# lsl036/STM-Multifrontal-QR-Factorization-Empowered-by-GCN

Measured on AMD Instinct MI355X. Metric: numerical-factorization GFLOP/s, higher is better.
Workload: dtype f64; 1 GPU; xenon1_colamd_standin: m=49248 n=49248 nnz=1258432 fronts=686 flops/step=5.029e+11, ordering default (COLAMD: qrtest without an ordering argument) (stand-in for xenon1.mtx, absent from the reference checkout); inputs=values resident in HBM, factors left in HBM, parallelism=replica x1, levels=16, retries=0

## Files before the change

### stm-multifrontal-qr-factorization-empowered-by-gcn_amd/csrc/stmmqr_update.hip

```cpp
#include <hip/hip_ext.h>
#include "stmmqr_kdev.h"
#include "stmmqr_knobs.h"


__global__ __launch_bounds__(NT) void k_update(DevCtx c, const int *__restrict__ flist, const int *__restrict__ plist, int cb0)
{
    extern __shared__ double dyn_lds[];
    const int f = flist[blockIdx.y];
    const int p = plist[blockIdx.y];
    const FrontSym s = c.fs[f];
    if (p >= s.npanels) return;
    const PanelDesc *pd = &c.fnum[f].pd[STM_PDI(p)];
    const int cbg = cb0 + (int)blockIdx.x * (1 + c.cbskip);
    const int c0 = pd->pc0 + cbg * BN;
    if (c0 >= s.fn) return;
    double *Tw = c.Tws + (long long)STM_TSLOT(c.tslot[f], p) * STM_NB * STM_NB;
    if (pd->t_deferred) {
        const bool first = (cbg == 0) || (c.cbskip > 0 && blockIdx.x == 0);
        dev_update_block(c.Farena + s.foff, s.ld, pd->pg1, pd->pt - pd->pg1, pd->pk1, pd->pnb, pd->pdiag, nullptr, c0,
                         min(BN, s.fn - c0), dyn_lds, c.Tau + s.rp + pd->pk1, first ? Tw : nullptr,
                         (first && c.Tall) ? c.Tall + (long long)(s.tpan + p) * STM_NB * STM_NB : nullptr);
        return;
    }
    dev_update_block(c.Farena + s.foff, s.ld, pd->pg1, pd->pt - pd->pg1, pd->pk1, pd->pnb, pd->pdiag, Tw, c0,
                     min(BN, s.fn - c0), dyn_lds);
}

__global__ __launch_bounds__(NT) void k_update_n(DevCtx c, int f)
{
    extern __shared__ double dyn_lds[];
    const FrontSym s = c.fs[f];
    const PanelDesc *pd = &c.fnum[f].pd[0];
    const int c0 = pd->pc0 + (int)blockIdx.x * BN;
    if (c0 >= s.fn) return;
    dev_update_block<true>(c.Farena + s.foff, s.ld, pd->pg1, pd->pt - pd->pg1, pd->pk1, pd->pnb, pd->pdiag,
                           c.Tws + STM_TSLOT(c.tslot[f], 0) * STM_NB * STM_NB, c0, min(BN, s.fn - c0), dyn_lds);
}

__global__ __launch_bounds__(NT) void k_larft(DevCtx c, int f)
{
    extern __shared__ double dyn_lds[];
    __shared__ PanelShared ps;
    int *s_diag = ps.diag;
    double *s_tau = ps.tau;
    double (*s_G)[STM_NB + 1] = ps.G;
    double (*s_T)[STM_NB + 1] = ps.T;
    const FrontSym s = c.fs[f];
    const PanelDesc *num = &c.fnum[f].pd[0];
    const int tid = threadIdx.x;
    if (tid < STM_NB) {
        s_diag[tid] = num->pdiag[tid];
        s_tau[tid] = (tid < num->pnb && num->pdiag[tid] != STM_BIGROW) ? c.Tau[s.rp + num->pk1 + tid] : 0.0;
    }
    __syncthreads();
    dev_gram_T<NT>(c.Farena + s.foff + (long long)num->pk1 * s.ld, s.ld, num->pg1, num->pt, num->pnb, s_diag, s_tau, s_G,
               s_T, c.Tws + STM_TSLOT(c.tslot[f], 0) * STM_NB * STM_NB, dyn_lds);
}


template <bool PRE = false>
__device__ __forceinline__ void dev_k_upd_w(const DevCtx &c, const int *__restrict__ flist, const int *__restrict__ plist, int cb0,
                                            int with_gram, double *Wp, const long long *__restrict__ wpoff, int *wcnt, int cb, int sl,
                                            int fi, int ncbx, double *dyn_lds)
{
    __shared__ int s_pd[STM_NB];
    const int f = flist[fi], p = plist[fi];
    const FrontSym s = c.fs[f];
    if (p >= s.npanels) return;
    const PanelDesc *pd = &c.fnum[f].pd[STM_PDI(p)];
    const int g1 = pd->pg1, mp = pd->pt - pd->pg1, nbp = pd->pnb;
    const int ncbf = stm_upd_ncb(s, p), nslf = stm_upd_nsl(s);
    const bool gram = with_gram && (cb == ncbx - 1);
    if ((c.dbg & 16) && c.dbgbuf && threadIdx.x == 0) {
        atomicAdd(&c.dbgbuf[40], 1ull);
        const int c0d = gram ? pd->pk1 : pd->pc0 + (cb0 + cb * (1 + c.cbskip)) * BN;
        if (!((gram && !pd->t_deferred) || (!gram && cb0 + cb * (1 + c.cbskip) >= ncbf) || nbp <= 0 || mp <= 0 || c0d >= s.fn || sl * SLAB >= mp))
            atomicAdd(&c.dbgbuf[41], 1ull);
    }
    if (gram && !pd->t_deferred) return;
    if (!gram && cb0 + cb * (1 + c.cbskip) >= ncbf) return;
    const int c0 = gram ? pd->pk1 : pd->pc0 + (cb0 + cb * (1 + c.cbskip)) * BN;
    if (nbp <= 0 || mp <= 0 || c0 >= s.fn || sl * SLAB >= mp) return;
    const int nc = gram ? nbp : min(BN, s.fn - c0);
    const long long ld = s.ld;
    const int tid = threadIdx.x, lane = tid & 63, wid = tid >> 6, l15 = lane & 15, l4 = lane >> 4;
    double *Vs = dyn_lds, *Cs = Vs + STM_NB * VS;
    if (tid < STM_NB) s_pd[tid] = (tid < nbp) ? pd->pdiag[tid] : STM_BIGROW;
    __syncthreads();
    const double *Vg = c.Farena + s.foff + g1 + (long long)pd->pk1 * ld;
    const double *Cg = c.Farena + s.foff + g1 + (long long)c0 * ld;
    const int mi = wid >> 1, ni = wid & 1;
    d4 acc = {0, 0, 0, 0};
    const int rend = min(mp, (sl + 1) * SLAB);
    if constexpr (PRE) {
        UpdChunk ckp[SLAB / RB];
#pragma unroll
        for (int q = 0; q < SLAB / RB; q++) upd_chunk_load(ckp[q], Vg, Cg, ld, sl * SLAB + q * RB + (tid & 63), mp, nbp, nc, tid >> 6);
        const int pfrom = (nc == BN) ? upd_plain_from(s_pd, g1, lane) : STM_BIGROW;
#pragma unroll
        for (int q = 0; q < SLAB / RB; q++) {
            const int r0 = sl * SLAB + q * RB;
            if (r0 < rend) {
                upd_chunk_to_lds(ckp[q], r0 + (tid & 63), mp, nbp, nc, s_pd, g1, tid & 63, tid >> 6, Vs, Cs, gram, r0 > pfrom && r0 + RB <= mp);
                __syncthreads();
#pragma unroll
                for (int kk = 0; kk < RB / 4; kk++) {
                    const double a = Vs[(16 * mi + l15) * VS + 4 * kk + l4];
                    const double b = Cs[(16 * ni + l15) * VS + 4 * kk + l4];
                    acc = __builtin_amdgcn_mfma_f64_16x16x4f64(a, b, acc, 0, 0, 0);
                }
                __syncthreads();
            }
        }
    } else {
    UpdChunk ck;
    upd_chunk_load(ck, Vg, Cg, ld, sl * SLAB + (tid & 63), mp, nbp, nc, tid >> 6);
    const int pfrom = (nc == BN) ? upd_plain_from(s_pd, g1, lane) : STM_BIGROW;
    for (int r0 = sl * SLAB; r0 < rend; r0 += RB) {
        upd_chunk_to_lds(ck, r0 + (tid & 63), mp, nbp, nc, s_pd, g1, tid & 63, tid >> 6, Vs, Cs, gram, r0 > pfrom && r0 + RB <= mp);
        __syncthreads();
        if (r0 + RB < rend) upd_chunk_load(ck, Vg, Cg, ld, r0 + RB + (tid & 63), mp, nbp, nc, tid >> 6);
#pragma unroll
        for (int kk = 0; kk < RB / 4; kk++) {
            const double a = Vs[(16 * mi + l15) * VS + 4 * kk + l4];
            const double b = Cs[(16 * ni + l15) * VS + 4 * kk + l4];
            acc = __builtin_amdgcn_mfma_f64_16x16x4f64(a, b, acc, 0, 0, 0);
        }
        __syncthreads();
    }
    }
    const int gslot = (c.ypoff && c.ypoff[f] >= 0) ? min(ncbf, c.sweep) : ncbf;
    double *W = Wp + wpoff[fi] + ((long long)(gram ? gslot : cb) * nslf + sl) * (STM_NB * BN);
    __shared__ int s_ticket;
    const int nsl = (mp + SLAB - 1) / SLAB;
    if (!gram) {
        if (nsl == 1) {
#pragma unroll
            for (int r = 0; r < 4; r++) W[(16 * mi + l4 + 4 * r) * BN + 16 * ni + l15] = acc[r];
            return;
        }
#pragma unroll
        for (int r = 0; r < 4; r++) st_agent(&W[(16 * mi + l4 + 4 * r) * BN + 16 * ni + l15], acc[r]);
        asm volatile("s_waitcnt vmcnt(0)" ::: "memory");
        __syncthreads();
        int *cnt = wcnt + wpoff[fi] / (STM_NB * BN) + cb;
        if (tid == 0) {
            s_ticket = __hip_atomic_fetch_add(cnt, 1, __ATOMIC_RELAXED, __HIP_MEMORY_SCOPE_AGENT);
            if (s_ticket == nsl - 1) {
                __builtin_amdgcn_fence(__ATOMIC_ACQUIRE, "agent");
                asm volatile("s_waitcnt vmcnt(0)" ::: "memory");
                __hip_atomic_store(cnt, 0, __ATOMIC_RELAXED, __HIP_MEMORY_SCOPE_AGENT);
            }
        }
        __syncthreads();
        if (s_ticket != nsl - 1) return;
        double *W0 = Wp + wpoff[fi] + ((long long)cb * nslf) * (STM_NB * BN);
        double v[STM_NB * BN / NT];
#pragma unroll
        for (int q = 0; q < STM_NB * BN / NT; q++) v[q] = stm_ordered_sum<true>(W0 + tid + q * NT, STM_NB * BN, nsl);
#pragma unroll
        for (int q = 0; q < STM_NB * BN / NT; q++) W0[tid + q * NT] = v[q];
        return;
    }
#pragma unroll
    for (int r = 0; r < 4; r++) st_agent(&W[(16 * mi + l4 + 4 * r) * BN + 16 * ni + l15], acc[r]);
    asm volatile("s_waitcnt vmcnt(0)" ::: "memory");
    __syncthreads();
    FrontNum *num = &c.fnum[f];
    if (tid == 0) {
        s_ticket = __hip_atomic_fetch_add(&num->gcnt, 1, __ATOMIC_RELAXED, __HIP_MEMORY_SCOPE_AGENT);
        if (s_ticket == nsl - 1) {
            __builtin_amdgcn_fence(__ATOMIC_ACQUIRE, "agent");
            asm volatile("s_waitcnt vmcnt(0)" ::: "memory");
            __hip_atomic_store(&num->gcnt, 0, __ATOMIC_RELAXED, __HIP_MEMORY_SCOPE_AGENT);
        }
    }
    __syncthreads();
    if (s_ticket != nsl - 1) return;
    double *s_G = Vs;
    __shared__ double s_tau[STM_NB];
    const double *G0 = Wp + wpoff[fi] + ((long long)gslot * nslf) * (STM_NB * BN);
    if (tid < STM_NB) s_tau[tid] = (tid < nbp) ? c.Tau[s.rp + pd->pk1 + tid] : 0.0;
    for (int e = tid; e < STM_NB * BN; e += NT) {
        const double gsum = stm_ordered_sum<false>(G0 + e, STM_NB * BN, nsl);
        s_G[(e / BN) * WS + (e % BN)] = gsum;
    }
    __syncthreads();
    double *Tout = c.Tws + (long long)STM_TSLOT(c.tslot[f], p) * STM_NB * STM_NB;
    double *Tkeep = c.Tall ? c.Tall + (long long)(s.tpan + p) * STM_NB * STM_NB : nullptr;
    double (*s_Tb)[STM_NB + 1] = reinterpret_cast<double (*)[STM_NB + 1]>(Cs);
    dev_T_from_gram(reinterpret_cast<double (*)[STM_NB + 1]>(s_G), s_Tb, s_tau, nbp, threadIdx.x);
    for (int e = tid; e < STM_NB * STM_NB; e += NT) {
        const int a = e % STM_NB, b = e / STM_NB;
        const double tv = (a <= b && a < nbp && b < nbp) ? s_Tb[a][b] : 0.0;
        Tout[e] = tv;
        if (Tkeep) Tkeep[e] = tv;
    }
}

__global__ __launch_bounds__(NT) void k_upd_w(DevCtx c, const int *__restrict__ flist, const int *__restrict__ plist, int cb0,
                                              int with_gram, double *Wp, const long long *__restrict__ wpoff, int *wcnt)
{
    extern __shared__ double dyn_lds[];
    dev_k_upd_w(c, flist, plist, cb0, with_gram, Wp, wpoff, wcnt, blockIdx.x, blockIdx.y, blockIdx.z, gridDim.x, dyn_lds);
}

__global__ __launch_bounds__(NT) void k_upd_c(DevCtx c, const int *__restrict__ flist, const int *__restrict__ plist, int cb0,
                                              const double *Wp, const long long *__restrict__ wpoff)
{
    extern __shared__ double dyn_lds[];
    __shared__ int s_pd[STM_NB];
    const int fi = blockIdx.z, f = flist[fi], p = plist[fi];
    const FrontSym s = c.fs[f];
    if (p >= s.npanels) return;
    const PanelDesc *pd = &c.fnum[f].pd[STM_PDI(p)];
    const int g1 = pd->pg1, mp = pd->pt - pd->pg1, nbp = pd->pnb;
    const int cb = blockIdx.x, sl = blockIdx.y;
    const int nslf = stm_upd_nsl(s);
    const int c0 = pd->pc0 + (cb0 + cb * (1 + c.cbskip)) * BN;
    if (nbp <= 0 || mp <= 0 || c0 >= s.fn || sl * SLAB >= mp) return;
    const int nsl_all = (mp + SLAB - 1) / SLAB;
    const int spw = (nsl_all >= 32) ? 4 : (nsl_all >= 16) ? 2 : 1;
    if (sl % spw) return;
    const int nc = min(BN, s.fn - c0);
    const long long ld = s.ld;
    const int tid = threadIdx.x, lane = tid & 63, wid = tid >> 6, l15 = lane & 15, l4 = lane >> 4;
    double *Vs = dyn_lds, *Cs = Vs + STM_NB * VS, *Ws = Cs + BN * VS;
    double *s_W1 = Vs, *s_T = Cs;
    if (tid < STM_NB) s_pd[tid] = (tid < nbp) ? pd->pdiag[tid] : STM_BIGROW;
    const double *Vg = c.Farena + s.foff + g1 + (long long)pd->pk1 * ld;
    double *Cg = c.Farena + s.foff + g1 + (long long)c0 * ld;
    const int lrow = tid & 63, lcg = tid >> 6;
    UpdChunk ck;
    upd_chunk_load(ck, Vg, Cg, ld, sl * SLAB + lrow, mp, nbp, nc, lcg);
    {
        const double *W0 = Wp + wpoff[fi] + ((long long)cb * nslf) * (STM_NB * BN);
        const double *T = c.Tws + (long long)STM_TSLOT(c.tslot[f], p) * STM_NB * STM_NB;
        for (int e = tid; e < STM_NB * BN; e += NT) {
            const double v = W0[e];
            s_W1[(e / BN) * WS + (e % BN)] = v;
            s_T[(e / STM_NB) * WS + (e % STM_NB)] = T[e];
        }
        __syncthreads();
        const d4 w2 = dev_w2_tile(s_T, 1, WS, s_W1, wid, lane);
#pragma unroll
        for (int r = 0; r < 4; r++) Ws[(16 * (wid >> 1) + l4 + 4 * r) * WS + 16 * (wid & 1) + l15] = w2[r];
    }
    __syncthreads();
    const int rend = min(mp, (sl + spw) * SLAB);
    const int pfrom = upd_plain_from(s_pd, g1, tid & 63);
    for (int r0 = sl * SLAB; r0 < rend; r0 += RB) {
        const int i = r0 + lrow;
        double cc[8];
#pragma unroll
        for (int q = 0; q < 8; q++) cc[q] = ck.c[q];
        upd_chunk_v_to_lds(ck, i, mp, nbp, s_pd, g1, lrow, lcg, Vs, r0 > pfrom && r0 + RB <= mp);
        __syncthreads();
        if (r0 + RB < rend) upd_chunk_load(ck, Vg, Cg, ld, i + RB, mp, nbp, nc, lcg);
        d4 u0 = {0, 0, 0, 0}, u1 = {0, 0, 0, 0};
#pragma unroll
        for (int kk = 0; kk < STM_NB / 4; kk++) {
            const double a = Vs[(4 * kk + l4) * VS + 16 * wid + l15];
            const double b0 = Ws[(4 * kk + l4) * WS + l15];
            const double b1 = Ws[(4 * kk + l4) * WS + 16 + l15];
            u0 = __builtin_amdgcn_mfma_f64_16x16x4f64(a, b0, u0, 0, 0, 0);
            u1 = __builtin_amdgcn_mfma_f64_16x16x4f64(a, b1, u1, 0, 0, 0);
        }
#pragma unroll
        for (int r = 0; r < 4; r++) {
            const int row = 16 * wid + l4 + 4 * r;
            Cs[l15 * VS + row] = u0[r];
            Cs[(16 + l15) * VS + row] = u1[r];
        }
        __syncthreads();
        if (i < mp) {
#pragma unroll
            for (int q = 0; q < 8; q++) {
                const int col = lcg * 8 + q;
                if (col < nc) Cg[i + col * ld] = cc[q] - Cs[col * VS + lrow];
            }
        }
    }
}

__device__ __forceinline__ void dev_k_upd_f(const DevCtx &c, const int *__restrict__ flist, const int *__restrict__ plist, int cb0,
                                            int with_gram, double *Wp, const long long *__restrict__ wpoff, int *wcnt, int *wflag,
                                            int epoch, int sl, int by, int fi, double *dyn_lds)
{
    __shared__ int s_pd[STM_NB];
    __shared__ int s_ticket, s_ok;
    const int f = flist[fi], p = plist[fi];
    const FrontSym s = c.fs[f];
    if (p >= s.npanels) return;
    FrontNum *num = &c.fnum[f];
    const PanelDesc *pd = &num->pd[STM_PDI(p)];
    const int g1 = pd->pg1, mp = pd->pt - pd->pg1, nbp = pd->pnb;
    const bool gram = with_gram && by == 0;
    const int cb = by - (with_gram ? 1 : 0);
    const int ncbf = stm_upd_ncb(s, p), nslf = stm_upd_nsl(s);
    if (gram && !pd->t_deferred) return;
    if (!gram && cb0 + cb * (1 + c.cbskip) >= ncbf) return;
    const int c0 = gram ? pd->pk1 : pd->pc0 + (cb0 + cb * (1 + c.cbskip)) * BN;
    if (nbp <= 0 || mp <= 0 || c0 >= s.fn || sl * SLAB >= mp) return;
    const int nc = gram ? nbp : min(BN, s.fn - c0);
    const long long ld = s.ld;
    const int tid = threadIdx.x, lane = tid & 63, wid = tid >> 6, l15 = lane & 15, l4 = lane >> 4;
    const int lrow = tid & 63, lcg = tid >> 6;
    double *Vs = dyn_lds, *Cs = Vs + STM_NB * VS, *Ws = Cs + BN * VS;
    if (tid < STM_NB) s_pd[tid] = (tid < nbp) ? pd->pdiag[tid] : STM_BIGROW;
    const double *Vg = c.Farena + s.foff + g1 + (long long)pd->pk1 * ld;
    double *Cg = c.Farena + s.foff + g1 + (long long)c0 * ld;
    const int r00 = sl * SLAB, rend = min(mp, (sl + 1) * SLAB);
    UpdChunk ck[SLAB / RB];
#pragma unroll
    for (int q = 0; q < SLAB / RB; q++) upd_chunk_load(ck[q], Vg, Cg, ld, r00 + q * RB + lrow, mp, nbp, nc, lcg);
    __syncthreads();
    const int mi = wid >> 1, ni = wid & 1;
    d4 acc = {0, 0, 0, 0};
#pragma unroll
    for (int q = 0; q < SLAB / RB; q++) {
        const int r0 = r00 + q * RB;
        if (r0 < rend) {
            upd_chunk_to_lds(ck[q], r0 + lrow, mp, nbp, nc, s_pd, g1, lrow, lcg, Vs, Cs, gram);
            __syncthreads();
#pragma unroll
            for (int kk = 0; kk < RB / 4; kk++) {
                const double a = Vs[(16 * mi + l15) * VS + 4 * kk + l4];
                const double b = Cs[(16 * ni + l15) * VS + 4 * kk + l4];
                acc = __builtin_amdgcn_mfma_f64_16x16x4f64(a, b, acc, 0, 0, 0);
            }
            __syncthreads();
        }
    }
    const int nsl = (mp + SLAB - 1) / SLAB;
    const int gslot = (c.ypoff && c.ypoff[f] >= 0) ? min(ncbf, c.sweep) : ncbf;
    double *Wslot = Wp + wpoff[fi] + ((long long)(gram ? gslot : cb) * nslf) * (STM_NB * BN);
    double *W = Wslot + (long long)sl * (STM_NB * BN);
#pragma unroll
    for (int r = 0; r < 4; r++) st_agent(&W[(16 * mi + l4 + 4 * r) * BN + 16 * ni + l15], acc[r]);
    asm volatile("s_waitcnt vmcnt(0)" ::: "memory");
    __syncthreads();
    double *Tslot = c.Tws + (long long)STM_TSLOT(c.tslot[f], p) * STM_NB * STM_NB;
    if (gram) {
        if (tid == 0) {
            s_ticket = __hip_atomic_fetch_add(&num->gcnt, 1, __ATOMIC_RELAXED, __HIP_MEMORY_SCOPE_AGENT);
            if (s_ticket == nsl - 1) {
                __builtin_amdgcn_fence(__ATOMIC_ACQUIRE, "agent");
                asm volatile("s_waitcnt vmcnt(0)" ::: "memory");
                __hip_atomic_store(&num->gcnt, 0, __ATOMIC_RELAXED, __HIP_MEMORY_SCOPE_AGENT);
            }
        }
        __syncthreads();
        if (s_ticket != nsl - 1) return;
        double *s_G = Vs;
        __shared__ double s_tau[STM_NB];
        if (tid < STM_NB) s_tau[tid] = (tid < nbp) ? c.Tau[s.rp + pd->pk1 + tid] : 0.0;
        for (int e = tid; e < STM_NB * BN; e += NT) {
            const double gsum = stm_ordered_sum<true>(Wslot + e, STM_NB * BN, nsl);
            s_G[(e / BN) * WS + (e % BN)] = gsum;
        }
        __syncthreads();
        double *Tkeep = c.Tall ? c.Tall + (long long)(s.tpan + p) * STM_NB * STM_NB : nullptr;
        double (*s_Tb)[STM_NB + 1] = reinterpret_cast<double (*)[STM_NB + 1]>(Cs);
        dev_T_from_gram(reinterpret_cast<double (*)[STM_NB + 1]>(s_G), s_Tb, s_tau, nbp, threadIdx.x);
        for (int e = tid; e < STM_NB * STM_NB; e += NT) {
            const int a = e % STM_NB, b = e / STM_NB;
            const double tv = (a <= b && a < nbp && b < nbp) ? s_Tb[a][b] : 0.0;
            st_agent(&Tslot[e], tv);
            if (Tkeep) Tkeep[e] = tv;
        }
        asm volatile("s_waitcnt vmcnt(0)" ::: "memory");
        __syncthreads();
        if (tid == 0) st_agent(&num->tready, epoch);
        return;
    }
    int *cnt = wcnt + wpoff[fi] / (STM_NB * BN) + cb;
    int *flag = wflag + wpoff[fi] / (STM_NB * BN) + cb;
    bool last = (nsl == 1);
    if (nsl > 1) {
        if (tid == 0) {
            s_ticket = __hip_atomic_fetch_add(cnt, 1, __ATOMIC_RELAXED, __HIP_MEMORY_SCOPE_AGENT);
            if (s_ticket == nsl - 1) {
                __builtin_amdgcn_fence(__ATOMIC_ACQUIRE, "agent");
                asm volatile("s_waitcnt vmcnt(0)" ::: "memory");
                __hip_atomic_store(cnt, 0, __ATOMIC_RELAXED, __HIP_MEMORY_SCOPE_AGENT);
            }
        }
        __syncthreads();
        last = (s_ticket == nsl - 1);
    }
    double *s_W1 = Vs, *s_T = Cs;
    if (last) {
        if (pd->t_deferred && !stm_wait_ge(&num->tready, epoch, c.abort, &s_ok)) { if (tid == 0) STM_SET_PERR(c, num); return; }
        for (int e = tid; e < STM_NB * BN; e += NT) {
            const double v = stm_ordered_sum<true>(Wslot + e, STM_NB * BN, nsl);
            s_W1[(e / BN) * WS + (e % BN)] = v;
            s_T[(e / STM_NB) * WS + (e % STM_NB)] = ld_agent(&Tslot[e]);
        }
        __syncthreads();
        const d4 w2 = dev_w2_tile(s_T, 1, WS, s_W1, wid, lane);
#pragma unroll
        for (int r = 0; r < 4; r++) Ws[(16 * (wid >> 1) + l4 + 4 * r) * WS + 16 * (wid & 1) + l15] = w2[r];
        if (nsl > 1) {
#pragma unroll
            for (int r = 0; r < 4; r++) st_agent(&Wslot[(16 * (wid >> 1) + l4 + 4 * r) * BN + 16 * (wid & 1) + l15], w2[r]);
            asm volatile("s_waitcnt vmcnt(0)" ::: "memory");
            __syncthreads();
            if (tid == 0) st_agent(flag, epoch);
        } else
            __syncthreads();
    } else {
        if (!stm_wait_ge(flag, epoch, c.abort, &s_ok)) { if (tid == 0) STM_SET_PERR(c, num); return; }
        for (int e = tid; e < STM_NB * BN; e += NT) Ws[(e / BN) * WS + (e % BN)] = ld_agent(&Wslot[e]);
        __syncthreads();
    }
#pragma unroll
    for (int q = 0; q < SLAB / RB; q++) {
        const int r0 = r00 + q * RB;
        if (r0 < rend) {
            const int i = r0 + lrow;
            upd_chunk_to_lds(ck[q], i, mp, nbp, nc, s_pd, g1, lrow, lcg, Vs, Cs);
            __syncthreads();
            d4 u0 = {0, 0, 0, 0}, u1 = {0, 0, 0, 0};
#pragma unroll
            for (int kk = 0; kk < STM_NB / 4; kk++) {
                const double a = Vs[(4 * kk + l4) * VS + 16 * wid + l15];
                const double b0 = Ws[(4 * kk + l4) * WS + l15];
                const double b1 = Ws[(4 * kk + l4) * WS + 16 + l15];
                u0 = __builtin_amdgcn_mfma_f64_16x16x4f64(a, b0, u0, 0, 0, 0);
                u1 = __builtin_amdgcn_mfma_f64_16x16x4f64(a, b1, u1, 0, 0, 0);
            }
#pragma unroll
            for (int r = 0; r < 4; r++) {
                const int row = 16 * wid + l4 + 4 * r;
                Cs[l15 * VS + row] -= u0[r];
                Cs[(16 + l15) * VS + row] -= u1[r];
            }
            __syncthreads();
            if (i < mp) {
#pragma unroll
                for (int qq = 0; qq < 8; qq++) {
                    const int col = lcg * 8 + qq;
                    if (col < nc) Cg[i + col * ld] = Cs[col * VS + lrow];
                }
            }
            __syncthreads();
        }
    }
}

__global__ __launch_bounds__(NT, 2) void k_upd_f(DevCtx c, const int *__restrict__ flist, const int *__restrict__ plist, int cb0,
                                              int with_gram, double *Wp, const long long *__restrict__ wpoff, int *wcnt,
                                              int *wflag, int epoch)
{
    extern __shared__ double dyn_lds[];
    dev_k_upd_f(c, flist, plist, cb0, with_gram, Wp, wpoff, wcnt, wflag, epoch, blockIdx.x, blockIdx.y, blockIdx.z, dyn_lds);
}

__device__ __forceinline__ void dev_k_upd_b0(const DevCtx &c, const int *__restrict__ flist, const int *__restrict__ plist, double *Wp,
                                             const long long *__restrict__ wpoff, int *wcnt, int *wflag, int epoch, int sl, int fi,
                                             double *dyn_lds)
{
    __shared__ int s_pd[STM_NB];
    __shared__ int s_ticket, s_ok;
    __shared__ double s_tau[STM_NB];
    const bool tl = (c.dbg & 32768) && c.dbgbuf && threadIdx.x == 0 && sl == 0;
    unsigned long long tl0 = tl ? wall_clock64() : 0;
#define B0TL(k) do { if (tl) { const unsigned long long t1 = wall_clock64(); atomicAdd(&c.dbgbuf[48 + (k)], t1 - tl0); tl0 = t1; } } while (0)
    const int f = flist[fi], p = plist[fi];
    const FrontSym s = c.fs[f];
    if (p >= s.npanels) return;
    FrontNum *num = &c.fnum[f];
    const PanelDesc *pd = &num->pd[STM_PDI(p)];
    const int g1 = pd->pg1, mp = pd->pt - pd->pg1, nbp = pd->pnb;
    const int ncbf = stm_upd_ncb(s, p), nslf = stm_upd_nsl(s);
    if (ncbf <= 0) return;
    const int c0 = pd->pc0;
    if (nbp <= 0 || mp <= 0 || c0 >= s.fn || sl * SLAB >= mp) return;
    const bool deferred = pd->t_deferred != 0;
    const int nc = min(BN, s.fn - c0);
    const long long ld = s.ld;
    const int tid = threadIdx.x, lane = tid & 63, wid = tid >> 6, l15 = lane & 15, l4 = lane >> 4;
    const int lrow = tid & 63, lcg = tid >> 6;
    double *Vs = dyn_lds, *Cs = Vs + STM_NB * VS, *Ws = Cs + BN * VS;
    if (tid < STM_NB) {
        s_pd[tid] = (tid < nbp) ? pd->pdiag[tid] : STM_BIGROW;
        s_tau[tid] = (tid < nbp) ? c.Tau[s.rp + pd->pk1 + tid] : 0.0;
    }
    const double *Vg = c.Farena + s.foff + g1 + (long long)pd->pk1 * ld;
    double *Cg = c.Farena + s.foff + g1 + (long long)c0 * ld;
    const int r00 = sl * SLAB, rend = min(mp, (sl + 1) * SLAB);
    UpdChunk ck[SLAB / RB];
#pragma unroll
    for (int q = 0; q < SLAB / RB; q++) upd_chunk_load(ck[q], Vg, Cg, ld, r00 + q * RB + lrow, mp, nbp, nc, lcg);
    const int nsl = (mp + SLAB - 1) / SLAB;
    const int gslot = (c.ypoff && c.ypoff[f] >= 0) ? min(ncbf, c.sweep) : ncbf;
    double *Wslot = Wp + wpoff[fi];
    double *Gslot = Wp + wpoff[fi] + ((long long)gslot * nslf) * (STM_NB * BN);
    double *Tslot = c.Tws + (long long)STM_TSLOT(c.tslot[f], p) * STM_NB * STM_NB;
    __syncthreads();
    B0TL(0);
    const int mi = wid >> 1, ni = wid & 1;
    d4 acc = {0, 0, 0, 0}, accg = {0, 0, 0, 0};
#pragma unroll
    for (int q = 0; q < SLAB / RB; q++) {
        const int r0 = r00 + q * RB;
        if (r0 < rend) {
            upd_chunk_to_lds(ck[q], r0 + lrow, mp, nbp, nc, s_pd, g1, lrow, lcg, Vs, Cs);
            __syncthreads();
#pragma unroll
            for (int kk = 0; kk < RB / 4; kk++) {
                const double a = Vs[(16 * mi + l15) * VS + 4 * kk + l4];
                const double b = Cs[(16 * ni + l15) * VS + 4 * kk + l4];
                acc = __builtin_amdgcn_mfma_f64_16x16x4f64(a, b, acc, 0, 0, 0);
            }
            if (deferred) {
#pragma unroll
                for (int kk = 0; kk < RB / 4; kk++) {
                    const double a = Vs[(16 * mi + l15) * VS + 4 * kk + l4];
                    const double b = Vs[(16 * ni + l15) * VS + 4 * kk + l4];
                    accg = __builtin_amdgcn_mfma_f64_16x16x4f64(a, b, accg, 0, 0, 0);
                }
            }
            __syncthreads();
        }
    }
    double *s_G = Vs, *s_W1 = Vs + STM_NB * WS, *s_T = Cs;
    B0TL(1);
    bool last = true;
    if (nsl > 1) {
        double *W = Wslot + (long long)sl * (STM_NB * BN), *G = Gslot + (long long)sl * (STM_NB * BN);
#pragma unroll
        for (int r = 0; r < 4; r++) st_agent(&W[(16 * mi + l4 + 4 * r) * BN + 16 * ni + l15], acc[r]);
        if (deferred) {
#pragma unroll
            for (int r = 0; r < 4; r++) st_agent(&G[(16 * mi + l4 + 4 * r) * BN + 16 * ni + l15], accg[r]);
        }
        asm volatile("s_waitcnt vmcnt(0)" ::: "memory");
        __syncthreads();
        int *cnt = wcnt + wpoff[fi] / (STM_NB * BN);
        int *flag = wflag + wpoff[fi] / (STM_NB * BN);
        if (tid == 0) {
            s_ticket = __hip_atomic_fetch_add(cnt, 1, __ATOMIC_RELAXED, __HIP_MEMORY_SCOPE_AGENT);
            if (s_ticket == nsl - 1) {
                __hip_atomic_store(cnt, 0, __ATOMIC_RELAXED, __HIP_MEMORY_SCOPE_AGENT);
                st_agent(flag, epoch);
            }
        }
        __syncthreads();
        last = (s_ticket == nsl - 1);
        B0TL(2);
        if (!stm_wait_ge(flag, epoch, c.abort, &s_ok)) { if (tid == 0) STM_SET_PERR(c, num); return; }
        B0TL(3);
        for (int e = tid; e < STM_NB * BN; e += NT) {
            s_W1[(e / BN) * WS + (e % BN)] = stm_ordered_sum<true>(Wslot + e, STM_NB * BN, nsl);
            if (deferred) s_G[(e / BN) * WS + (e % BN)] = stm_ordered_sum<true>(Gslot + e, STM_NB * BN, nsl);
        }
    } else {
#pragma unroll
        for (int r = 0; r < 4; r++) {
            s_W1[(16 * mi + l4 + 4 * r) * WS + 16 * ni + l15] = acc[r];
            if (deferred) s_G[(16 * mi + l4 + 4 * r) * WS + 16 * ni + l15] = accg[r];
        }
    }
    __syncthreads();
    B0TL(4);
    double (*s_Tb)[STM_NB + 1] = reinterpret_cast<double (*)[STM_NB + 1]>(s_T);
    if (deferred) {
        dev_T_from_gram(reinterpret_cast<double (*)[STM_NB + 1]>(s_G), s_Tb, s_tau, nbp, tid);
        if (last) {
            double *Tkeep = c.Tall ? c.Tall + (long long)(s.tpan + p) * STM_NB * STM_NB : nullptr;
            for (int e = tid; e < STM_NB * STM_NB; e += NT) {
                const int a = e % STM_NB, b = e / STM_NB;
                const double tv = (a <= b && a < nbp && b < nbp) ? s_Tb[a][b] : 0.0;
                Tslot[e] = tv;
                if (Tkeep) Tkeep[e] = tv;
            }
        }
    } else {
        for (int e = tid; e < STM_NB * STM_NB; e += NT) s_Tb[e % STM_NB][e / STM_NB] = Tslot[e];
        __syncthreads();
    }
    B0TL(5);
    {
        const d4 w2 = dev_w2_tile(s_T, WS, 1, s_W1, wid, lane);
#pragma unroll
        for (int r = 0; r < 4; r++) Ws[(16 * (wid >> 1) + l4 + 4 * r) * WS + 16 * (wid & 1) + l15] = w2[r];
    }
    __syncthreads();
    B0TL(6);
#pragma unroll
    for (int q = 0; q < SLAB / RB; q++) {
        const int r0 = r00 + q * RB;
        if (r0 < rend) {
            const int i = r0 + lrow;
            upd_chunk_to_lds(ck[q], i, mp, nbp, nc, s_pd, g1, lrow, lcg, Vs, Cs);
            __syncthreads();
            d4 u0 = {0, 0, 0, 0}, u1 = {0, 0, 0, 0};
#pragma unroll
            for (int kk = 0; kk < STM_NB / 4; kk++) {
                const double a = Vs[(4 * kk + l4) * VS + 16 * wid + l15];
                const double b0 = Ws[(4 * kk + l4) * WS + l15];
                const double b1 = Ws[(4 * kk + l4) * WS + 16 + l15];
                u0 = __builtin_amdgcn_mfma_f64_16x16x4f64(a, b0, u0, 0, 0, 0);
                u1 = __builtin_amdgcn_mfma_f64_16x16x4f64(a, b1, u1, 0, 0, 0);
            }
#pragma unroll
            for (int r = 0; r < 4; r++) {
                const int row = 16 * wid + l4 + 4 * r;
                Cs[l15 * VS + row] -= u0[r];
                Cs[(16 + l15) * VS + row] -= u1[r];
            }
            __syncthreads();
            if (i < mp) {
#pragma unroll
                for (int qq = 0; qq < 8; qq++) {
                    const int col = lcg * 8 + qq;
                    if (col < nc) Cg[i + col * ld] = Cs[col * VS + lrow];
                }
            }
            __syncthreads();
        }
    }
    asm volatile("s_waitcnt vmcnt(0)" ::: "memory");
    B0TL(7);
    if (tl) atomicAdd(&c.dbgbuf[56], 1ull);
#undef B0TL
}

__device__ __forceinline__ void dev_upd_w_rider(const DevCtx &c, const int *__restrict__ flist, const int *__restrict__ plist, int cb0,
                                                double *Wp, const long long *__restrict__ wpoff, int *wcnt, int cb, int y, int rspw,
                                                int fi, double *dyn_lds)
{
    __shared__ int s_pd[STM_NB];
    __shared__ int s_ticket;
    const int f = flist[fi], p = plist[fi];
    const FrontSym s = c.fs[f];
    if (p >= s.npanels) return;
    const PanelDesc *pd = &c.fnum[f].pd[STM_PDI(p)];
    const int g1 = pd->pg1, mp = pd->pt - pd->pg1, nbp = pd->pnb;
    const int ncbf = stm_upd_ncb(s, p), nslf = stm_upd_nsl(s);
    if (cb0 + cb >= ncbf) return;
    const int c0 = pd->pc0 + (cb0 + cb) * BN;
    const int sl0 = y * rspw;
    if (nbp <= 0 || mp <= 0 || c0 >= s.fn || sl0 * SLAB >= mp) return;
    const int nc = min(BN, s.fn - c0);
    const long long ld = s.ld;
    const int tid = threadIdx.x, lane = tid & 63, wid = tid >> 6, l15 = lane & 15, l4 = lane >> 4;
    double *Vs = dyn_lds, *Cs = Vs + STM_NB * VS;
    if (tid < STM_NB) s_pd[tid] = (tid < nbp) ? pd->pdiag[tid] : STM_BIGROW;
    __syncthreads();
    const double *Vg = c.Farena + s.foff + g1 + (long long)pd->pk1 * ld;
    const double *Cg = c.Farena + s.foff + g1 + (long long)c0 * ld;
    const int mi = wid >> 1, ni = wid & 1;
    const int nsl = (mp + SLAB - 1) / SLAB;
    const int rend = min(mp, (sl0 + rspw) * SLAB);
    double *W = Wp + wpoff[fi] + ((long long)cb * nslf + sl0) * (STM_NB * BN);
    d4 acc = {0, 0, 0, 0};
    UpdChunk ck;
    upd_chunk_load(ck, Vg, Cg, ld, sl0 * SLAB + (tid & 63), mp, nbp, nc, tid >> 6);
    const int pfrom = (nc == BN) ? upd_plain_from(s_pd, g1, lane) : STM_BIGROW;
    int done = 0;
    for (int r0 = sl0 * SLAB; r0 < rend; r0 += RB) {
        upd_chunk_to_lds(ck, r0 + (tid & 63), mp, nbp, nc, s_pd, g1, tid & 63, tid >> 6, Vs, Cs, false, r0 > pfrom && r0 + RB <= mp);
        __syncthreads();
        if (r0 + RB < rend) upd_chunk_load(ck, Vg, Cg, ld, r0 + RB + (tid & 63), mp, nbp, nc, tid >> 6);
#pragma unroll
        for (int kk = 0; kk < RB / 4; kk++) {
            const double a = Vs[(16 * mi + l15) * VS + 4 * kk + l4];
            const double b = Cs[(16 * ni + l15) * VS + 4 * kk + l4];
            acc = __builtin_amdgcn_mfma_f64_16x16x4f64(a, b, acc, 0, 0, 0);
        }
        __syncthreads();
        if (((r0 + RB) % SLAB) == 0 || r0 + RB >= rend) {
            if (nsl == 1) {
#pragma unroll
                for (int r = 0; r < 4; r++) W[(16 * mi + l4 + 4 * r) * BN + 16 * ni + l15] = acc[r];
            } else {
#pragma unroll
                for (int r = 0; r < 4; r++) st_agent(&W[(16 * mi + l4 + 4 * r) * BN + 16 * ni + l15], acc[r]);
            }
            W += STM_NB * BN;
            acc = d4{0, 0, 0, 0};
            done++;
        }
    }
    if (nsl == 1) return;
    asm volatile("s_waitcnt vmcnt(0)" ::: "memory");
    __syncthreads();
    int *cnt = wcnt + wpoff[fi] / (STM_NB * BN) + cb;
    if (tid == 0) {
        s_ticket = __hip_atomic_fetch_add(cnt, done, __ATOMIC_RELAXED, __HIP_MEMORY_SCOPE_AGENT);
        if (s_ticket + done == nsl) {
            __builtin_amdgcn_fence(__ATOMIC_ACQUIRE, "agent");
            asm volatile("s_waitcnt vmcnt(0)" ::: "memory");
            __hip_atomic_store(cnt, 0, __ATOMIC_RELAXED, __HIP_MEMORY_SCOPE_AGENT);
        }
    }
    __syncthreads();
    if (s_ticket + done != nsl) return;
    double *W0 = Wp + wpoff[fi] + ((long long)cb * nslf) * (STM_NB * BN);
    double v[STM_NB * BN / NT];
#pragma unroll
    for (int q = 0; q < STM_NB * BN / NT; q++) v[q] = stm_ordered_sum<true>(W0 + tid + q * NT, STM_NB * BN, nsl);
#pragma unroll
    for (int q = 0; q < STM_NB * BN / NT; q++) W0[tid + q * NT] = v[q];
}

__global__ __launch_bounds__(NT, 2) void k_upd_b0w(DevCtx c, const int *__restrict__ flist, const int *__restrict__ plist, int nfr,
                                                   int maxsl, int ncbrest, double *Wp, const long long *__restrict__ wpoff, int *wcnt,
                                                   int *wflag, int epoch, double *Wp2, int *wcnt2, int rspw)
{
    extern __shared__ double dyn_lds[];
    if ((int)blockIdx.z < nfr) {
        if ((int)blockIdx.x >= maxsl || blockIdx.y >= 1) return;
        dev_k_upd_b0(c, flist, plist, Wp, wpoff, wcnt, wflag, epoch, blockIdx.x, blockIdx.z, dyn_lds);
        return;
    }
    if ((int)blockIdx.x >= ncbrest || (int)blockIdx.y * rspw >= maxsl) return;
    dev_upd_w_rider(c, flist, plist, 1, Wp2, wpoff, wcnt2, blockIdx.x, blockIdx.y, rspw, (int)blockIdx.z - nfr, dyn_lds);
}

__global__ __launch_bounds__(NT, 2) void k_upd_fw(DevCtx c, const int *__restrict__ flist, const int *__restrict__ plist, int nfr,
                                                  int maxsl, int ncbrest, double *Wp, const long long *__restrict__ wpoff, int *wcnt,
                                                  int *wflag, int epoch, double *Wp2, int *wcnt2)
{
    extern __shared__ double dyn_lds[];
    if ((int)blockIdx.z < nfr) {
        if ((int)blockIdx.x >= maxsl || blockIdx.y >= 2) return;
        dev_k_upd_f(c, flist, plist, 0, 1, Wp, wpoff, wcnt, wflag, epoch, blockIdx.x, blockIdx.y, blockIdx.z, dyn_lds);
        return;
    }
    if ((int)blockIdx.x >= ncbrest || (int)blockIdx.y >= maxsl) return;
    dev_k_upd_w<true>(c, flist, plist, 1, 0, Wp2, wpoff, wcnt2, blockIdx.x, blockIdx.y, (int)blockIdx.z - nfr, ncbrest, dyn_lds);
}
int stm_update_lds_bytes(void) { return (int)((2 * BN * VS + STM_NB * WS) * sizeof(double)); }
int stm_launch_update(const DevCtx &c, const int *flist, const int *plist, int nfr, int cb0, int ncb, hipStream_t st)
{
    if (nfr <= 0 || ncb <= 0) return 0;
    hipLaunchKernelGGL(k_update, dim3(ncb, nfr), dim3(NT), (size_t)stm_update_lds_bytes(), st, c, flist, plist, cb0);
    return (int)hipGetLastError();
}
int stm_launch_update_split(const DevCtx &c, const int *flist, const int *plist, int nfr, int cb0, int ncb, int maxsl, double *Wp,
                            const long long *wpoff, int *wcnt, int with_gram, hipStream_t st)
{
    if (nfr <= 0 || ncb + (with_gram ? 1 : 0) <= 0 || maxsl <= 0) return 0;
    const size_t lds = (size_t)stm_update_lds_bytes();
    hipLaunchKernelGGL(k_upd_w, dim3(ncb + (with_gram ? 1 : 0), maxsl, nfr), dim3(NT), (size_t)(2 * BN * VS) * sizeof(double), st, c,
                       flist, plist, cb0, with_gram ? 1 : 0, Wp, wpoff, wcnt);
    if (ncb > 0) hipLaunchKernelGGL(k_upd_c, dim3(ncb, maxsl, nfr), dim3(NT), lds, st, c, flist, plist, cb0, (const double *)Wp, wpoff);
    return (int)hipGetLastError();
}
int stm_launch_update_fused(const DevCtx &c, const int *flist, const int *plist, int nfr, int cb0, int ncb, int maxsl, double *Wp,
                            const long long *wpoff, int *wcnt, int *wflag, int epoch, int with_gram, hipStream_t st)
{
    const int ny = ncb + (with_gram ? 1 : 0);
    if (nfr <= 0 || ny <= 0 || maxsl <= 0) return 0;
    hipLaunchKernelGGL(k_upd_f, dim3(maxsl, ny, nfr), dim3(NT), (size_t)stm_update_lds_bytes(), st, c, flist, plist, cb0,
                       with_gram ? 1 : 0, Wp, wpoff, wcnt, wflag, epoch);
    return (int)hipGetLastError();
}
int stm_launch_update_fw(const DevCtx &c, const int *flist, const int *plist, int nfr, int ncb, int maxsl, double *Wp,
                         const long long *wpoff, int *wcnt, int *wflag, int epoch, double *Wp2, int *wcnt2, hipStream_t st)
{
    if (nfr <= 0 || maxsl <= 0) return 0;
    const int rest = ncb - 1;
    const int one = (int)knobs::once<knobs::K_B0_ONE>();
    if (one) {
        const int rspw = (int)knobs::once<knobs::K_RSPW_W>();
        const int uy = (maxsl + rspw - 1) / rspw;
        hipLaunchKernelGGL(k_upd_b0w, dim3(maxsl > rest ? maxsl : rest, rest > 0 ? uy : 1, rest > 0 ? 2 * nfr : nfr), dim3(NT),
                           (size_t)stm_update_lds_bytes(), st, c, flist, plist, nfr, maxsl, rest > 0 ? rest : 0, Wp, wpoff, wcnt, wflag, epoch,
                           Wp2, wcnt2, rspw);
        return (int)hipGetLastError();
    }
    if (rest <= 0) return stm_launch_update_fused(c, flist, plist, nfr, 0, 1, maxsl, Wp, wpoff, wcnt, wflag, epoch, 1, st);
    hipLaunchKernelGGL(k_upd_fw, dim3(maxsl > rest ? maxsl : rest, maxsl > 2 ? maxsl : 2, 2 * nfr), dim3(NT), (size_t)stm_update_lds_bytes(),
                       st, c, flist, plist, nfr, maxsl, rest, Wp, wpoff, wcnt, wflag, epoch, Wp2, wcnt2);
    return (int)hipGetLastError();
}
static int stm_anyorder(void)
{
    return (int)knobs::once<knobs::K_ANYORDER>();
}
int stm_launch_update_w(const DevCtx &c, const int *flist, const int *plist, int nfr, int cb0, int ncb, int maxsl, double *Wp,
                        const long long *wpoff, int *wcnt, hipStream_t st)
{
    if (nfr <= 0 || ncb <= 0 || maxsl <= 0) return 0;
    if (stm_anyorder())
        hipExtLaunchKernelGGL(k_upd_w, dim3(ncb, maxsl, nfr), dim3(NT), (size_t)(2 * BN * VS) * sizeof(double), st, nullptr, nullptr,
                              hipExtAnyOrderLaunch, c, flist, plist, cb0, 0, Wp, wpoff, wcnt);
    else
    hipLaunchKernelGGL(k_upd_w, dim3(ncb, maxsl, nfr), dim3(NT), (size_t)(2 * BN * VS) * sizeof(double), st, c, flist, plist, cb0, 0, Wp,
                       wpoff, wcnt);
    return (int)hipGetLastError();
}
int stm_launch_update_c(const DevCtx &c, const int *flist, const int *plist, int nfr, int cb0, int ncb, int maxsl, const double *Wp,
                        const long long *wpoff, hipStream_t st)
{
    if (nfr <= 0 || ncb <= 0 || maxsl <= 0) return 0;
    if (stm_anyorder())
        hipExtLaunchKernelGGL(k_upd_c, dim3(ncb, maxsl, nfr), dim3(NT), (size_t)stm_update_lds_bytes(), st, nullptr, nullptr,
                              hipExtAnyOrderLaunch, c, flist, plist, cb0, Wp, wpoff);
    else
    hipLaunchKernelGGL(k_upd_c, dim3(ncb, maxsl, nfr), dim3(NT), (size_t)stm_update_lds_bytes(), st, c, flist, plist, cb0, Wp, wpoff);
    return (int)hipGetLastError();
}
int stm_launch_update_notrans(const DevCtx &c, int f, int ncb, hipStream_t st)
{
    if (ncb <= 0) return 0;
    hipLaunchKernelGGL(k_update_n, dim3(ncb), dim3(NT), (size_t)stm_update_lds_bytes(), st, c, f);
    return (int)hipGetLastError();
}
int stm_launch_larft(const DevCtx &c, int f, hipStream_t st)
{
    hipLaunchKernelGGL(k_larft, dim3(1), dim3(NT), (size_t)stm_update_lds_bytes(), st, c, f);
    return (int)hipGetLastError();
}
int stm_configure_update(void)
{
    CK(hipFuncSetAttribute((const void *)k_update, hipFuncAttributeMaxDynamicSharedMemorySize, 65536));
    CK(hipFuncSetAttribute((const void *)k_update_n, hipFuncAttributeMaxDynamicSharedMemorySize, 65536));
    return 0;
}
```

Before: 5703 GFLOP/s.

## Double-buffer LDS chunks and batch metadata/ordered-sum loads in b0 update kernel

Reworks the panel-0 update kernel so that each chunk's V/C data is written to one of two LDS buffers while the MFMA loop consumes the other, removing a barrier per chunk. Front and panel descriptors are fetched with one word per lane and broadcast via readlane, replacing scalar struct loads. Cross-slab partial sums are now unrolled over several slabs and elements at once to raise memory-level parallelism. The C writeback subtracts the product from register-held C instead of doing a read-modify-write in LDS. The cost is a larger LDS footprint (four images), which may lower occupancy, and it needs a raised dynamic-LDS attribute.

```diff
diff --git a/stm-multifrontal-qr-factorization-empowered-by-gcn_amd/csrc/stmmqr_update.hip b/stm-multifrontal-qr-factorization-empowered-by-gcn_amd/csrc/stmmqr_update.hip
--- a/stm-multifrontal-qr-factorization-empowered-by-gcn_amd/csrc/stmmqr_update.hip
+++ b/stm-multifrontal-qr-factorization-empowered-by-gcn_amd/csrc/stmmqr_update.hip
@@ -457,6 +457,30 @@
     dev_k_upd_f(c, flist, plist, cb0, with_gram, Wp, wpoff, wcnt, wflag, epoch, blockIdx.x, blockIdx.y, blockIdx.z, dyn_lds);
 }
 
+#define STM_B0_LDS_DOUBLES (4 * BN * VS + STM_NB * WS)
+template <int K, int U>
+__device__ __forceinline__ void stm_ordered_sums(double (&v)[K], const double *const (&p)[K], long long stride, int n)
+{
+#pragma unroll
+    for (int k = 0; k < K; k++) v[k] = 0;
+    for (int q = 0; q < n; q += U) {
+        double t[K][U];
+#pragma unroll
+        for (int k = 0; k < K; k++) {
+#pragma unroll
+            for (int u = 0; u < U; u++) {
+                const double x = ld_agent(p[k] + (long long)min(q + u, n - 1) * stride);
+                t[k][u] = (q + u < n) ? x : 0.0;
+            }
+        }
+#pragma unroll
+        for (int k = 0; k < K; k++) {
+#pragma unroll
+            for (int u = 0; u < U; u++) v[k] += t[k][u];
+        }
+    }
+}
+
 __device__ __forceinline__ void dev_k_upd_b0(const DevCtx &c, const int *__restrict__ flist, const int *__restrict__ plist, double *Wp,
                                              const long long *__restrict__ wpoff, int *wcnt, int *wflag, int epoch, int sl, int fi,
                                              double *dyn_lds)
@@ -468,46 +492,64 @@
     unsigned long long tl0 = tl ? wall_clock64() : 0;
 #define B0TL(k) do { if (tl) { const unsigned long long t1 = wall_clock64(); atomicAdd(&c.dbgbuf[48 + (k)], t1 - tl0); tl0 = t1; } } while (0)
     const int f = flist[fi], p = plist[fi];
-    const FrontSym s = c.fs[f];
+    const int tid = threadIdx.x, lane = tid & 63, wid = tid >> 6, l15 = lane & 15, l4 = lane >> 4;
+    const int lrow = tid & 63, lcg = tid >> 6;
+    FrontNum *num = &c.fnum[f];
+    constexpr int FSW = (int)(sizeof(FrontSym) / sizeof(int)), PDW = (int)(offsetof(PanelDesc, pad3) / sizeof(int));
+    static_assert(FSW <= 64 && PDW <= 64 && offsetof(PanelDesc, pdiag) / sizeof(int) + STM_NB <= 64, "one word per lane");
+    const int wfs = ld_agent(reinterpret_cast<const int *>(&c.fs[f]) + min(lane, FSW - 1));
+    const int wpd = ld_agent(reinterpret_cast<const int *>(&num->pd[STM_PDI(p)]) + min(lane, PDW - 1));
+    const int tsl = ld_agent(&c.tslot[f]);
+    const long long wpo = wpoff[fi];
+    const long long ypl = __hip_atomic_load(c.ypoff ? &c.ypoff[f] : &wpoff[fi], __ATOMIC_RELAXED, __HIP_MEMORY_SCOPE_AGENT);
+    const bool pairf = c.ypoff && ypl >= 0;
+#define B0FS(field) __builtin_amdgcn_readlane(wfs, (int)(offsetof(FrontSym, field) / sizeof(int)))
+#define B0PD(field) __builtin_amdgcn_readlane(wpd, (int)(offsetof(PanelDesc, field) / sizeof(int)))
+    FrontSym s;
+    s.foff = (long long)(((unsigned long long)(unsigned)__builtin_amdgcn_readlane(wfs, (int)(offsetof(FrontSym, foff) / sizeof(int)) + 1) << 32) |
+                         (unsigned)B0FS(foff));
+    s.ld = B0FS(ld); s.fn = B0FS(fn); s.rp = B0FS(rp); s.fm_ub = B0FS(fm_ub); s.npanels = B0FS(npanels); s.tpan = B0FS(tpan);
+    const int g1 = B0PD(pg1), mp = B0PD(pt) - g1, pk1 = B0PD(pk1), nbp = B0PD(pnb), c0 = B0PD(pc0);
+    const bool deferred = B0PD(t_deferred) != 0;
+    const int pdv = __shfl(wpd, (int)(offsetof(PanelDesc, pdiag) / sizeof(int)) + (lane & (STM_NB - 1)));
+#undef B0FS
+#undef B0PD
     if (p >= s.npanels) return;
-    FrontNum *num = &c.fnum[f];
-    const PanelDesc *pd = &num->pd[STM_PDI(p)];
-    const int g1 = pd->pg1, mp = pd->pt - pd->pg1, nbp = pd->pnb;
     const int ncbf = stm_upd_ncb(s, p), nslf = stm_upd_nsl(s);
     if (ncbf <= 0) return;
-    const int c0 = pd->pc0;
     if (nbp <= 0 || mp <= 0 || c0 >= s.fn || sl * SLAB >= mp) return;
-    const bool deferred = pd->t_deferred != 0;
     const int nc = min(BN, s.fn - c0);
     const long long ld = s.ld;
-    const int tid = threadIdx.x, lane = tid & 63, wid = tid >> 6, l15 = lane & 15, l4 = lane >> 4;
-    const int lrow = tid & 63, lcg = tid >> 6;
-    double *Vs = dyn_lds, *Cs = Vs + STM_NB * VS, *Ws = Cs + BN * VS;
+    auto img = [&](int k) { return dyn_lds + k * (BN * VS); };
+    double *Ws = dyn_lds + 4 * BN * VS;
+    const double tauv = ld_agent(&c.Tau[s.rp + pk1 + min(lane & (STM_NB - 1), nbp - 1)]);
+    const double *Vg = c.Farena + s.foff + g1 + (long long)pk1 * ld;
+    double *Cg = c.Farena + s.foff + g1 + (long long)c0 * ld;
+    const int r00 = sl * SLAB, nch = (min(mp, (sl + 1) * SLAB) - r00 + RB - 1) / RB;
+    const int nsl = (mp + SLAB - 1) / SLAB;
+    const int gslot = pairf ? min(ncbf, c.sweep) : ncbf;
+    const long long goff = wpo + ((long long)gslot * nslf) * (STM_NB * BN);
+    auto Wslot = [&] { return Wp + wpo; };
+    auto Gslot = [&] { return Wp + goff; };
+    auto Tslot = [&] { return c.Tws + (long long)STM_TSLOT(tsl, p) * STM_NB * STM_NB; };
+    UpdChunk ck[SLAB / RB];
+#pragma unroll
+    for (int q = 0; q < SLAB / RB; q++) upd_chunk_load(ck[q], Vg, Cg, ld, r00 + q * RB + lrow, mp, nbp, nc, lcg);
     if (tid < STM_NB) {
-        s_pd[tid] = (tid < nbp) ? pd->pdiag[tid] : STM_BIGROW;
-        s_tau[tid] = (tid < nbp) ? c.Tau[s.rp + pd->pk1 + tid] : 0.0;
-    }
-    const double *Vg = c.Farena + s.foff + g1 + (long long)pd->pk1 * ld;
-    double *Cg = c.Farena + s.foff + g1 + (long long)c0 * ld;
-    const int r00 = sl * SLAB, rend = min(mp, (sl + 1) * SLAB);
-    UpdChunk ck[SLAB / RB];
-#pragma unroll
-    for (int q = 0; q < SLAB / RB; q++) upd_chunk_load(ck[q], Vg, Cg, ld, r00 + q * RB + lrow, mp, nbp, nc, lcg);
-    const int nsl = (mp + SLAB - 1) / SLAB;
-    const int gslot = (c.ypoff && c.ypoff[f] >= 0) ? min(ncbf, c.sweep) : ncbf;
-    double *Wslot = Wp + wpoff[fi];
-    double *Gslot = Wp + wpoff[fi] + ((long long)gslot * nslf) * (STM_NB * BN);
-    double *Tslot = c.Tws + (long long)STM_TSLOT(c.tslot[f], p) * STM_NB * STM_NB;
+        s_pd[tid] = (tid < nbp) ? pdv : STM_BIGROW;
+        s_tau[tid] = (tid < nbp) ? tauv : 0.0;
+    }
     __syncthreads();
     B0TL(0);
     const int mi = wid >> 1, ni = wid & 1;
     d4 acc = {0, 0, 0, 0}, accg = {0, 0, 0, 0};
+    upd_chunk_to_lds(ck[0], r00 + lrow, mp, nbp, nc, s_pd, g1, lrow, lcg, img(0), img(1));
+    __syncthreads();
 #pragma unroll
     for (int q = 0; q < SLAB / RB; q++) {
         const int r0 = r00 + q * RB;
-        if (r0 < rend) {
-            upd_chunk_to_lds(ck[q], r0 + lrow, mp, nbp, nc, s_pd, g1, lrow, lcg, Vs, Cs);
-            __syncthreads();
+        if (q < nch) {
+            const double *Vs = img(2 * (q & 1)), *Cs = img(2 * (q & 1) + 1);
 #pragma unroll
             for (int kk = 0; kk < RB / 4; kk++) {
                 const double a = Vs[(16 * mi + l15) * VS + 4 * kk + l4];
@@ -522,14 +564,17 @@
                     accg = __builtin_amdgcn_mfma_f64_16x16x4f64(a, b, accg, 0, 0, 0);
                 }
             }
+            if (q + 1 < nch)
+                upd_chunk_to_lds(ck[(q + 1) % (SLAB / RB)], r0 + RB + lrow, mp, nbp, nc, s_pd, g1, lrow, lcg, img(2 * ((q + 1) & 1)),
+                                 img(2 * ((q + 1) & 1) + 1));
             __syncthreads();
         }
     }
-    double *s_G = Vs, *s_W1 = Vs + STM_NB * WS, *s_T = Cs;
+    double *s_G = img(0), *s_W1 = img(0) + STM_NB * WS, *s_T = img(1);
     B0TL(1);
     bool last = true;
     if (nsl > 1) {
-        double *W = Wslot + (long long)sl * (STM_NB * BN), *G = Gslot + (long long)sl * (STM_NB * BN);
+        double *W = Wslot() + (long long)sl * (STM_NB * BN), *G = Gslot() + (long long)sl * (STM_NB * BN);
 #pragma unroll
         for (int r = 0; r < 4; r++) st_agent(&W[(16 * mi + l4 + 4 * r) * BN + 16 * ni + l15], acc[r]);
         if (deferred) {
@@ -552,9 +597,30 @@
         B0TL(2);
         if (!stm_wait_ge(flag, epoch, c.abort, &s_ok)) { if (tid == 0) STM_SET_PERR(c, num); return; }
         B0TL(3);
-        for (int e = tid; e < STM_NB * BN; e += NT) {
-            s_W1[(e / BN) * WS + (e % BN)] = stm_ordered_sum<true>(Wslot + e, STM_NB * BN, nsl);
-            if (deferred) s_G[(e / BN) * WS + (e % BN)] = stm_ordered_sum<true>(Gslot + e, STM_NB * BN, nsl);
+        constexpr int NE = STM_NB * BN / NT;
+        if (deferred) {
+            const double *pp[2 * NE];
+            double v[2 * NE];
+#pragma unroll
+            for (int k = 0; k < NE; k++) { pp[k] = Wslot() + tid + k * NT; pp[NE + k] = Gslot() + tid + k * NT; }
+            stm_ordered_sums<2 * NE, 4>(v, pp, STM_NB * BN, nsl);
+#pragma unroll
+            for (int k = 0; k < NE; k++) {
+                const int e = tid + k * NT;
+                s_W1[(e / BN) * WS + (e % BN)] = v[k];
+                s_G[(e / BN) * WS + (e % BN)] = v[NE + k];
+            }
+        } else {
+            const double *pp[NE];
+            double v[NE];
+#pragma unroll
+            for (int k = 0; k < NE; k++) pp[k] = Wslot() + tid + k * NT;
+            stm_ordered_sums<NE, 8>(v, pp, STM_NB * BN, nsl);
+#pragma unroll
+            for (int k = 0; k < NE; k++) {
+                const int e = tid + k * NT;
+                s_W1[(e / BN) * WS + (e % BN)] = v[k];
+            }
         }
     } else {
 #pragma unroll
@@ -573,29 +639,33 @@
             for (int e = tid; e < STM_NB * STM_NB; e += NT) {
                 const int a = e % STM_NB, b = e / STM_NB;
                 const double tv = (a <= b && a < nbp && b < nbp) ? s_Tb[a][b] : 0.0;
-                Tslot[e] = tv;
+                Tslot()[e] = tv;
                 if (Tkeep) Tkeep[e] = tv;
             }
         }
     } else {
-        for (int e = tid; e < STM_NB * STM_NB; e += NT) s_Tb[e % STM_NB][e / STM_NB] = Tslot[e];
+        for (int e = tid; e < STM_NB * STM_NB; e += NT) s_Tb[e % STM_NB][e / STM_NB] = Tslot()[e];
         __syncthreads();
     }
     B0TL(5);
     {
+        upd_chunk_v_to_lds(ck[0], r00 + lrow, mp, nbp, s_pd, g1, lrow, lcg, img(2));
         const d4 w2 = dev_w2_tile(s_T, WS, 1, s_W1, wid, lane);
 #pragma unroll
         for (int r = 0; r < 4; r++) Ws[(16 * (wid >> 1) + l4 + 4 * r) * WS + 16 * (wid & 1) + l15] = w2[r];
     }
     __syncthreads();
     B0TL(6);
+    const int nch2 = wave_uniform(nch);
 #pragma unroll
     for (int q = 0; q < SLAB / RB; q++) {
         const int r0 = r00 + q * RB;
-        if (r0 < rend) {
+        if (q < nch2) {
             const int i = r0 + lrow;
-            upd_chunk_to_lds(ck[q], i, mp, nbp, nc, s_pd, g1, lrow, lcg, Vs, Cs);
-            __syncthreads();
+            const double *Vs = img(2 * ((q + 1) & 1));
+            double *Ps = img(2 * ((q + 1) & 1) + 1);
+            if (q + 1 < nch2)
+                upd_chunk_v_to_lds(ck[(q + 1) % (SLAB / RB)], i + RB, mp, nbp, s_pd, g1, lrow, lcg, img(2 * (q & 1)));
             d4 u0 = {0, 0, 0, 0}, u1 = {0, 0, 0, 0};
 #pragma unroll
             for (int kk = 0; kk < STM_NB / 4; kk++) {
@@ -608,18 +678,17 @@
 #pragma unroll
             for (int r = 0; r < 4; r++) {
                 const int row = 16 * wid + l4 + 4 * r;
-                Cs[l15 * VS + row] -= u0[r];
-                Cs[(16 + l15) * VS + row] -= u1[r];
+                Ps[l15 * VS + row] = u0[r];
+                Ps[(16 + l15) * VS + row] = u1[r];
             }
             __syncthreads();
             if (i < mp) {
 #pragma unroll
                 for (int qq = 0; qq < 8; qq++) {
                     const int col = lcg * 8 + qq;
-                    if (col < nc) Cg[i + col * ld] = Cs[col * VS + lrow];
+                    if (col < nc) Cg[i + col * ld] = ck[q].c[qq] - Ps[col * VS + lrow];
                 }
             }
-            __syncthreads();
         }
     }
     asm volatile("s_waitcnt vmcnt(0)" ::: "memory");
@@ -735,6 +804,7 @@
     dev_k_upd_w<true>(c, flist, plist, 1, 0, Wp2, wpoff, wcnt2, blockIdx.x, blockIdx.y, (int)blockIdx.z - nfr, ncbrest, dyn_lds);
 }
 int stm_update_lds_bytes(void) { return (int)((2 * BN * VS + STM_NB * WS) * sizeof(double)); }
+static size_t stm_update_b0_lds_bytes(void) { return (size_t)STM_B0_LDS_DOUBLES * sizeof(double); }
 int stm_launch_update(const DevCtx &c, const int *flist, const int *plist, int nfr, int cb0, int ncb, hipStream_t st)
 {
     if (nfr <= 0 || ncb <= 0) return 0;
@@ -770,7 +840,7 @@
         const int rspw = (int)knobs::once<knobs::K_RSPW_W>();
         const int uy = (maxsl + rspw - 1) / rspw;
         hipLaunchKernelGGL(k_upd_b0w, dim3(maxsl > rest ? maxsl : rest, rest > 0 ? uy : 1, rest > 0 ? 2 * nfr : nfr), dim3(NT),
-                           (size_t)stm_update_lds_bytes(), st, c, flist, plist, nfr, maxsl, rest > 0 ? rest : 0, Wp, wpoff, wcnt, wflag, epoch,
+                           stm_update_b0_lds_bytes(), st, c, flist, plist, nfr, maxsl, rest > 0 ? rest : 0, Wp, wpoff, wcnt, wflag, epoch,
                            Wp2, wcnt2, rspw);
         return (int)hipGetLastError();
     }
@@ -821,5 +891,6 @@
 {
     CK(hipFuncSetAttribute((const void *)k_update, hipFuncAttributeMaxDynamicSharedMemorySize, 65536));
     CK(hipFuncSetAttribute((const void *)k_update_n, hipFuncAttributeMaxDynamicSharedMemorySize, 65536));
+    CK(hipFuncSetAttribute((const void *)k_upd_b0w, hipFuncAttributeMaxDynamicSharedMemorySize, (int)stm_update_b0_lds_bytes()));
     return 0;
 }
```

Result: faster. 5822 GFLOP/s, median of 6 (+2.1%).
